# Martinsos/edlib

Measured on AMD Instinct MI355X. Metric: GCUPS (cell updates/s), 1M x 150bp HW reads vs 5Mb target, higher is better.
Workload: dtype u32

## Files before the change

edlib_amd/csrc/engine.hpp:

```cpp
#pragma once
#include "../../include/edlib_amd.h"
#include "common.hpp"
#include "pair_kernels.hpp"
#include "lanepair.hpp"
#include "reads_kernels.hpp"
#include "cross_kernels.hpp"
#include "window_kernels.hpp"
#include "strands.hpp"
#include "flat_pairs_prepare.hpp"
#include "pairs_gather.hpp"

#include <chrono>
#include <deque>
#include <functional>
#include <memory>
#include <vector>

namespace edlib_amd {

struct Tables {
    uint8_t tlut[256];
    uint8_t idToByte[256];
    int sigmaT = 0;
    uint32_t presence[8];
// ... 201 lines not shown
        DevBuf<int> d_best, d_total, d_pos, d_flags;
        DevBuf<uint32_t> d_peq;
        bool zeroCopy = false; PinBuf hostOut;
        std::vector<int> ovfSlots; std::vector<long long> ovfOff; DevBuf<int> d_ovfPool;
        DevBuf<int> d_lvMap, d_lvBest, d_lvCnt, d_lvPos; std::vector<int> lvMap; int lvS = 0, lvCap = 0; bool lvValid = false;
        DevBuf<int> d_list;
        int nreal = -1;
        bool mates = false; DevBuf<int> d_win;
    };
    static constexpr int kLastLevelCap = 16;
    int listOpenSlots(ReadGroup& g, int kDone, std::vector<int>& out);
    DevBuf<uint8_t> d_selTmp_;
    std::vector<std::unique_ptr<ReadGroup>> groups_;
    DevBuf<uint32_t> d_tpk_, d_trows_;
    DevBuf<unsigned long long> d_wordSteps_;
    PinBuf h_wordSteps_; bool wordStepsPending_ = false;
    DevBuf<unsigned long long> d_ringSteps_; PinBuf h_ringSteps_; bool ringStepsUsed_ = false;
    unsigned long long* ringStepsCounter();
    bool banded_ = false;
    int syms_ = 4;
    int packTarget();
    int runReads();
    int makeGroup(const std::vector<int>& units, int words, std::unique_ptr<ReadGroup>& g, long long oneRoundWaves = 0);
    int runGroupScans(ReadGroup& g, bool fullOnly);
    int runGroupExact(ReadGroup& g);
    int collectGroup(ReadGroup& g, std::vector<UnitResult>& res);
    int seedThreshold(const ReadGroup& g, bool fullOnly) const;
    int buildSeedIndex();
    int runSeedPass(ReadGroup& g, int k);
    DevBuf<uint32_t> d_seedCnt_, d_seedOff_, d_seedPos_;
    DevBuf<uint8_t> d_seedTmp_;
    bool hits_ = false, hitsHaveRun_ = false;
    HitListBuffers hitList_;
    HitRows hostHits_;
    DevBuf<int> d_hitSlotUnit_;
    DevBuf<long long> d_hitTotal_;
    int runReadHits();
    int scanGroupHits(ReadGroup& g, int slotBase);
    int hitsScanBanded(ReadGroup& g, int slotBase, const int* d_slotmap, int nlanes, int numSegments, int segLen, int warm);
    struct Piece { long long off; int len; int thr; };
    int scanPieces(const std::vector<Piece>& pieces, bool filter, std::vector<std::pair<int, int>>* cand,
                   std::vector<uint8_t>* overflow, std::vector<int>* best);
    int solveLongReads(std::vector<UnitResult>& res, std::vector<int>& fallback);
    bool filterScan_ = false;
    struct ChainArgs { const uint32_t* in = nullptr; uint32_t* out = nullptr; const int* src = nullptr; int inLanes = 0, blocks = 0; const int* rowBase = nullptr; };
    ChainArgs chain_;
    int solveTallFull(const std::vector<int>& units, std::vector<UnitResult>& res, std::vector<int>& handBack);
    int collectReads(std::vector<UnitResult>& res);
    bool readsCollected_ = true;
    int scanGroup(ReadGroup& g, int mode, const int* d_slotmap, int nlanes, int kcap, const int* d_kinit,
                  int numSegments, int segLen, int warm, int* segBest, int* segCnt, int* segPos, int cap,
                  const long long* posOff, const int* posCap, bool unbanded = false,
                  unsigned long long* wordSteps = nullptr, const uint32_t* peqDense = nullptr,
                  const int* qlenDense = nullptr, int peqBottom = 0, int* liveBest = nullptr);

    DevBuf<PairDesc> d_descs_;
    DevBuf<unsigned long long> d_peq64_;
    DevBuf<StoreEntry> d_store_;
    DevBuf<int> d_aux_, d_out3_, d_outScore_, d_outCount_, d_outLast_, d_posPool_, d_opsLen_, d_alpha_;
    DevBuf<uint8_t> d_ops_;
    DevBuf<long long> d_opsOff_;
    int solve(int mode, bool wantPositions, bool wantPath, const std::vector<UnitSpec>& units, SolveOut& out,
              int ring = 0, int ringH = 1);
    int solveChunk(int mode, bool wantPositions, bool wantPath, const std::vector<UnitSpec>& units,
                   size_t a, size_t b, SolveOut& out, int ring, int ringH);
    static const int kWide = -1;
    static const int kRing32 = -2;
    bool ring32_fits(const std::vector<UnitSpec>& units, size_t a, size_t b, int G) const;
    DevBuf<unsigned long long> d_wide_; DevBuf<unsigned> d_wabort_; PinBuf h_wabort_;
    int wideCap_ = -1;
    struct WidePlan { int slots = 1; size_t perLaunch = 1; };
    int planWide(int mode, PairDesc* descs, size_t n, WidePlan& plan);
    int launchWide(int mode, const PairScanArgs& a, const PairDesc* hostDescs, size_t n, const WidePlan& plan);
    int checkWide();
    bool wideSerial_ = false;
    bool wideGateHeld_ = false;
    void wideGateRelease();
    int solveWideSplit(const std::vector<UnitSpec>& units, std::vector<int>& out, int ring = 0);
    struct KnownSplit { long long qoff; int m; long long toff; int T; int score; int row, left, right; };
    std::vector<KnownSplit> knownSplits_;
    int solveGlobalDistances(const std::vector<UnitSpec>& units, std::vector<int>& score, std::vector<OpsOut>* paths = nullptr);
    int solveSemiGlobal(int mode, bool wantPositions, const std::vector<UnitSpec>& units, SolveOut& out);
    int solveSemiGlobalUnits(int mode, bool wantPositions, const std::vector<UnitSpec>& units, SolveOut& out);
    int solveBanded(const BandLadder& ladder, bool wantPositions, const std::vector<UnitSpec>& units, SolveOut& out);
    int alphabetLengthsBegin(hipEvent_t after = nullptr);
    bool alphaDeferred_ = false;
    int alphabetLengthsEnd(std::vector<UnitResult>& res);
    std::vector<int> alphaUnits_; bool alphaOnHost_ = false, alphaPending_ = false; long long alphaBytes_ = 0;
    hipStream_t side_ = nullptr;
    DevBuf<int> d_alphaIdx_, d_alphaOut_; PinBuf alphaPin_;
    struct PathPiece { long long qoff; int m; long long toff; int T; int score; };
    int hirschbergLevel(const std::vector<PathPiece>& big, std::vector<int>& splitRow,
                        std::vector<int>& leftScore, std::vector<int>& rightScore);
    int solvePaths(const std::vector<PathPiece>& jobs, std::vector<OpsOut>& opsOut, std::vector<int>& status);
    std::vector<std::shared_ptr<PinBuf>> opsKeep_;
    std::deque<std::vector<uint8_t>> opsOwned_;

    int qlen(int u) const { return (int)(qoff_[u + 1] - qoff_[u]); }
    long long tbase(int u) const { return shared_ ? toff_[0] : toff_[u]; }
    int tlen(int u) const { return shared_ ? (int)(toff_[1] - toff_[0]) : (int)(toff_[u + 1] - toff_[u]); }

    void scanTimerStart();
    void scanTimerStop();
    std::vector<std::pair<hipEvent_t, hipEvent_t>> scanEvents_;
    size_t scanEventsUsed_ = 0;

    std::vector<UnitResult> results_, work_;
// ... 151 lines not shown
```

edlib_amd/csrc/engine_reads.hip:

```cpp
#include "engine.hpp"

#include <algorithm>
#include <chrono>
#include <cmath>
#include <condition_variable>
#include <cstring>
#include <mutex>
#include <thread>

namespace edlib_amd {

__global__ void __launch_bounds__(256)
seed_thresholds_kernel(int* __restrict__ kinit, const int* __restrict__ best, const int* __restrict__ cnt, int n)
{
    const int i = blockIdx.x * blockDim.x + threadIdx.x;
    if (i < n && cnt[i] > 0 && best[i] < kinit[i]) kinit[i] = best[i];
}


int Batch::scanGroup(ReadGroup& g, int mode, const int* d_slotmap, int nlanes, int kcap, const int* d_kinit,
                     int numSegments, int segLen, int warm, int* segBest, int* segCnt, int* segPos, int cap,
                     const long long* posOff, const int* posCap, bool unbanded, unsigned long long* wordSteps,
                     const uint32_t* peqDense, const int* qlenDense, int peqBottom, int* liveBest)
{
    ReadScanArgs a{};
    a.peq = peqDense ? peqDense : g.d_peq.p; a.tpk = d_tpk_.p; a.trows = d_trows_.p; a.targetLength = tlen(0);
    if (mode == EDLIB_MODE_SHW) a.targetLength = (int)std::min<long long>(a.targetLength, 64LL * g.nwords + 1);
    a.qlen = qlenDense ? qlenDense : g.d_qlen.p; a.kinit = d_kinit; a.slotmap = d_slotmap; a.nlanes = nlanes;
    a.numSegments = numSegments; a.segLen = segLen; a.warm = warm;
    a.segBest = segBest; a.segCnt = segCnt; a.segPos = segPos; a.cap = cap;
    a.posOff = posOff; a.posCap = posCap;
    a.kcap = kcap; a.wordSteps = wordSteps ? wordSteps : d_wordSteps_.p;
    a.filter = filterScan_ ? 1 : 0;
    a.liveBest = liveBest;
    a.bottomAligned = peqBottom;
    a.chainIn = chain_.in; a.chainOut = chain_.out; a.chainSrc = chain_.src; a.chainInLanes = chain_.inLanes;
    a.chainBlocks = chain_.blocks; a.rowBase = chain_.rowBase;
    const bool chained = chain_.in != nullptr || chain_.out != nullptr;
    static const bool dbg = getenv("EDLIB_AMD_DEBUG") != nullptr;
    if (dbg) {
        EDLIB_AMD_HIP(hipStreamSynchronize(stream_));
        fprintf(stderr, "[edlib_amd] scanGroup nwords=%d mode=%d nlanes=%d S=%d segLen=%d warm=%d cap=%d kcap=%d slotmap=%p posOff=%p rows=%s\n",
                g.nwords, mode, nlanes, numSegments, segLen, warm, cap, kcap, (const void*)d_slotmap, (const void*)posOff,
                peqBottom > 1 ? "delay" : (peqBottom ? "bottom" : "top"));
    }
    scanTimerStart();
    const bool longGroup = g.nwords > kMaxReadWords;
    const long long colsScanned = std::min<long long>(a.targetLength, (long long)numSegments * segLen) + (long long)(numSegments - 1) * warm;
    const bool fullHeight = banded_ && mode == EDLIB_MODE_HW && unbanded && (chained || syms_ > 4 || longGroup);
    const bool bandedKernel = !fullHeight && banded_ && mode == EDLIB_MODE_HW && (!unbanded || syms_ > 4 || longGroup);
    if (peqBottom && (fullHeight || bandedKernel)) EDLIB_AMD_HIP(hipErrorInvalidValue);
    if (fullHeight) {
        EDLIB_AMD_HIP(launch_scan_reads_full(g.nwords, syms_, a, stream_));
        stats.word_steps += (long long)((nlanes + 63) / 64 * 64) * g.nwords * colsScanned;
    } else if (bandedKernel) EDLIB_AMD_HIP(launch_scan_reads_banded(g.nwords, syms_, a, stream_));
    else {
        EDLIB_AMD_HIP(launch_scan_reads(g.nwords, mode, a, stream_));
        stats.word_steps += (long long)((nlanes + 63) / 64 * 64) * g.nwords * colsScanned;
    }
    scanTimerStop();
    if (dbg) {
        EDLIB_AMD_HIP(hipStreamSynchronize(stream_));
        fprintf(stderr, "[edlib_amd] scanGroup done\n");
    }
    return 0;
}

void plan_segments(int nlanes, int T, int mode, int warmFull, long long wantWaves,
                          int& S, int& segLen, int& warm, int minSegCols)
{
    S = 1; segLen = roundup(T, 16); warm = 0;
    if (mode != EDLIB_MODE_HW) return;
    const long long nrblk = ((long long)nlanes + 63) / 64;
    long long want = (wantWaves + nrblk - 1) / nrblk;
    want = std::max(1LL, std::min<long long>(want, std::min(65535, std::max(1, T / minSegCols))));
    if (warmFull > 0) want = std::max(1LL, std::min<long long>(want, std::max<long long>(1, T / (4LL * warmFull))));
    segLen = roundup((int)((T + want - 1) / want), 16);
    S = (T + segLen - 1) / segLen;
    warm = warmFull;
}

int Batch::runReads()
{
    if (groups_.empty()) return 0;
    stats.path |= 1;
    bool seed = false;
    for (auto& gp : groups_) seed = seed || seedThreshold(*gp, false) >= 0;
    if (seed && buildSeedIndex()) return 1;
    for (auto& gp : groups_) if (runGroupScans(*gp, false)) return 1;
    const int mode = (cfg_.mode == EDLIB_MODE_HW || cfg_.mode == EDLIB_MODE_SHW) ? (int)cfg_.mode : (int)EDLIB_MODE_NW;
    for (auto& gp : groups_)
        if (gp->mates) EDLIB_AMD_HIP(launch_resolve_strands(gp->d_perm.p, gp->d_best.p, gp->d_total.p, gp->nslots, mode, cfg_.k,
                                                            gp->d_win.p, stream_));
    for (auto& gp : groups_) if (runGroupExact(*gp)) return 1;
    return 0;
}

int Batch::runGroupScans(ReadGroup& g, bool fullOnly)
{
    const int T = tlen(0);
    const int mode = (cfg_.mode == EDLIB_MODE_HW || cfg_.mode == EDLIB_MODE_SHW) ? (int)cfg_.mode : (int)EDLIB_MODE_NW;
    const bool banded = banded_ && mode == EDLIB_MODE_HW;
    const int kNoCap = 0x3fffffff;
    static const bool dbgLadder = getenv("EDLIB_AMD_DEBUG") != nullptr;
    EDLIB_AMD_HIP(launch_build_peq_reads(g.nwords, syms_, d_qpool_.p, d_qoff_.p, g.d_perm.p, g.nslots,
                                         d_eqtbl_.p, d_presence_.p, cfg_.k, g.d_peq.p, g.d_qlen.p,
                                         g.d_kinit.p, g.d_alphaExtra.p, stream_));
    const int kSeed = seedThreshold(g, fullOnly);
    const int kFirstMax = kSeed >= 0 ? kSeed : std::max(8, g.nwords / 2);
    int kFirst = (kSeed >= 0 && cfg_.k >= 0) ? std::min(kSeed, cfg_.k) : kFirstMax;
    bool twoPass = !fullOnly && banded && (cfg_.k < 0 || cfg_.k > kFirst) && 32 * g.nwords > kFirst;
    std::vector<int> ladder;
    g.lvValid = false;
    auto probe_scan = [&](const std::vector<int>& map, int kc, std::vector<int>& bestOut) -> int {
        const int nm = (int)map.size();
        int S2, segLen2, warm2;
        plan_segments(nm, T, mode, g.warm, 16384, S2, segLen2, warm2);
        const size_t items = (size_t)nm * S2;
        DevBuf<int> d_map, d_sb, d_sc;
        EDLIB_AMD_HIP(d_map.alloc(nm)); EDLIB_AMD_HIP(d_sb.alloc(items)); EDLIB_AMD_HIP(d_sc.alloc(items));
        EDLIB_AMD_HIP(hipMemcpyAsync(d_map.p, map.data(), nm * sizeof(int), hipMemcpyHostToDevice, stream_));
        if (scanGroup(g, mode, d_map.p, nm, kc, g.d_kinit.p, S2, segLen2, warm2,
                      d_sb.p, d_sc.p, d_sb.p , 0, nullptr, nullptr)) return 1;
        std::vector<int> cnts(items), bests(items);
        EDLIB_AMD_HIP(hipMemcpyAsync(cnts.data(), d_sc.p, items * sizeof(int), hipMemcpyDeviceToHost, stream_));
        EDLIB_AMD_HIP(hipMemcpyAsync(bests.data(), d_sb.p, items * sizeof(int), hipMemcpyDeviceToHost, stream_));
        EDLIB_AMD_HIP(hipStreamSynchronize(stream_));
        bestOut.assign(nm, -1);
        for (int i = 0; i < nm; ++i) {
            int b = 0x7fffffff;
            for (int sg = 0; sg < S2; ++sg)
                if (cnts[(size_t)i * S2 + sg] > 0) b = std::min(b, bests[(size_t)i * S2 + sg]);
// ... 41 lines not shown
        if (probe_scan(probe, kFirst, pbest)) return 1;
        int resolved = 0, real = 0;
        std::vector<int> hist(kFirstMax + 1, 0);
        std::vector<int> open;
        for (int i = 0; i < np; ++i) {
            if (g.perm[probe[i]] < 0) continue;
            ++real;
            if (pbest[i] >= 0) { ++resolved; ++hist[pbest[i]]; }
            else if (i == 0 || probe[i] != probe[i - 1]) open.push_back(probe[i]);
        }
        if (resolved > 0) {
            int acc = 0, kq = kFirstMax;
            for (int d = 0; d <= kFirstMax; ++d) { acc += hist[d]; if (acc * 1000LL >= resolved * 995LL) { kq = d; break; } }
            kFirst = std::max(4, std::min(kFirstMax, kq));
        }
        if (real > 0 && resolved * 10 < real * 3) twoPass = false;
        if (twoPass && (int)open.size() * 10 > real && open.size() >= 32 && price_ladder(open, open.size(), real)) return 1;
    }
    std::vector<int> todo;
    bool haveTodo = false;
    if (kSeed >= 0) {
        if (runSeedPass(g, kFirst)) return 1;
        if (twoPass) {
            if (listOpenSlots(g, kFirst, todo)) return 1;
            haveTodo = true;
            if (g.nreal < 0) { g.nreal = 0; for (int u : g.perm) g.nreal += u >= 0; }
            if (g.nslots >= 16384 && todo.size() * 10 > (size_t)g.nreal && todo.size() >= 32) {
                const size_t nsm = std::min<size_t>(2048, todo.size());
                std::vector<int> sample(nsm);
                for (size_t i = 0; i < nsm; ++i) sample[i] = todo[i * todo.size() / nsm];
                if (price_ladder(sample, todo.size(), g.nreal)) return 1;
            }
        }
    } else {
        if (scanGroup(g, mode, nullptr, g.nslots, twoPass ? kFirst : kNoCap, g.d_kinit.p, g.numSegments, g.segLen,
                      g.warm, g.d_segBest.p, g.d_segCnt.p, g.d_segPos.p, 8, nullptr, nullptr, fullOnly)) return 1;
        const bool chained = chain_.in != nullptr || chain_.out != nullptr;
        EDLIB_AMD_HIP(launch_merge_segments(g.d_segBest.p, g.d_segCnt.p, g.d_segPos.p, g.numSegments, 8,
                                            g.nslots, nullptr, 16, g.d_best.p, g.d_total.p, g.d_pos.p,
                                            g.d_flags.p, stream_, chained ? kOvfRescan : kOvfGatherGroup));
    }
    ladder.push_back(kNoCap);
    int kDone = kFirst;
    for (size_t lv = 0; twoPass && lv < ladder.size(); ++lv) {
        const int kcapL = ladder[lv];
        const bool last = kcapL == kNoCap;
        if (!haveTodo && listOpenSlots(g, kDone, todo)) return 1;
        haveTodo = false;
        if (todo.empty()) break;
        {
            const size_t no = todo.size();
            int S2, segLen2, warm2;
            plan_segments((int)no, T, mode, g.warm, 65536, S2, segLen2, warm2);
            const size_t items = no * (size_t)S2;
            const int capL = last ? kLastLevelCap : 8;
            EDLIB_AMD_HIP(g.d_lvMap.ensure(no)); EDLIB_AMD_HIP(g.d_lvBest.ensure(items)); EDLIB_AMD_HIP(g.d_lvCnt.ensure(items));
            EDLIB_AMD_HIP(g.d_lvPos.ensure(items * capL));
            int *d_map = g.d_lvMap.p, *d_sb = g.d_lvBest.p, *d_sc = g.d_lvCnt.p, *d_sp = g.d_lvPos.p;
            EDLIB_AMD_HIP(hipMemcpyAsync(d_map, todo.data(), no * sizeof(int), hipMemcpyHostToDevice, stream_));
            bool plain = false;
            if (last && no >= 4096) {
                const int np2 = 64;
                std::vector<int> sub(np2);
                for (int i = 0; i < np2; ++i) sub[i] = todo[(size_t)((long long)i * no / np2)];
                int S3, segLen3, warm3;
                plan_segments(np2, T, mode, g.warm, 16384, S3, segLen3, warm3);
                const size_t it3 = (size_t)np2 * S3;
                DevBuf<int> d_m3, d_b3, d_c3, d_p3; DevBuf<unsigned long long> d_ws;
                EDLIB_AMD_HIP(d_m3.alloc(np2)); EDLIB_AMD_HIP(d_b3.alloc(it3)); EDLIB_AMD_HIP(d_c3.alloc(it3));
                EDLIB_AMD_HIP(d_p3.alloc(it3 * 8)); EDLIB_AMD_HIP(d_ws.alloc(1));
                EDLIB_AMD_HIP(hipMemcpyAsync(d_m3.p, sub.data(), np2 * sizeof(int), hipMemcpyHostToDevice, stream_));
                EDLIB_AMD_HIP(hipMemsetAsync(d_ws.p, 0, sizeof(unsigned long long), stream_));
                if (scanGroup(g, mode, d_m3.p, np2, kNoCap, g.d_kinit.p, S3, segLen3, warm3,
                              d_b3.p, d_c3.p, d_p3.p, 8, nullptr, nullptr, false, d_ws.p)) return 1;
                unsigned long long ws = 0;
                EDLIB_AMD_HIP(hipMemcpyAsync(&ws, d_ws.p, sizeof ws, hipMemcpyDeviceToHost, stream_));
                EDLIB_AMD_HIP(hipStreamSynchronize(stream_));
                const double cols = (double)np2 * ((double)T + (double)(S3 - 1) * warm3);
                plain = (double)ws >= 0.85 * g.nwords * cols;
                stats.word_steps += (long long)ws;
            }
            const bool bottomOk = plain && mode == EDLIB_MODE_HW && syms_ == 4 && g.nwords <= kMaxReadWords &&
                                  chain_.in == nullptr && chain_.out == nullptr;
            const int bottom = !bottomOk ? 0 : (delay_rows_fit(g.nwords, g.mMax) ? 1 + kDelayRows : 1);
            const size_t no64 = (no + 63) / 64 * 64;
            std::vector<int> perm2(no64, -1);
            for (size_t i = 0; i < no; ++i) perm2[i] = g.perm[todo[i]];
            DevBuf<int> d_perm2, d_qlen2, d_kinit2, d_extra2; DevBuf<uint32_t> d_peq2;
            EDLIB_AMD_HIP(d_perm2.alloc(no64)); EDLIB_AMD_HIP(d_qlen2.alloc(no64)); EDLIB_AMD_HIP(d_kinit2.alloc(no64));
            EDLIB_AMD_HIP(d_extra2.alloc(no64)); EDLIB_AMD_HIP(d_peq2.alloc(no64 * (size_t)syms_ * g.nwords));
            EDLIB_AMD_HIP(hipMemcpyAsync(d_perm2.p, perm2.data(), no64 * sizeof(int), hipMemcpyHostToDevice, stream_));
            EDLIB_AMD_HIP(launch_build_peq_reads(g.nwords, syms_, d_qpool_.p, d_qoff_.p, d_perm2.p, (int)no64,
                                                 d_eqtbl_.p, d_presence_.p, cfg_.k, d_peq2.p, d_qlen2.p,
                                                 d_kinit2.p, d_extra2.p, stream_, bottom));
            const int seedCols = 4096;
            DevBuf<int> d_b0, d_c0, d_p0;
            if (mode == EDLIB_MODE_HW && last && no >= 4096 && S2 > 1 && T >= 16 * seedCols) {
                EDLIB_AMD_HIP(d_b0.alloc(no)); EDLIB_AMD_HIP(d_c0.alloc(no)); EDLIB_AMD_HIP(d_p0.alloc(no * 8));
                if (scanGroup(g, mode, nullptr, (int)no, kcapL, d_kinit2.p, 1, seedCols, 0,
                              d_b0.p, d_c0.p, d_p0.p, 8, nullptr, nullptr, plain, nullptr, d_peq2.p, d_qlen2.p, bottom)) return 1;
                hipLaunchKernelGGL(seed_thresholds_kernel, dim3((unsigned)((no + 255) / 256)), dim3(256), 0, stream_,
                                   d_kinit2.p, d_b0.p, d_c0.p, (int)no);
                EDLIB_AMD_HIP(hipGetLastError());
            }
            DevBuf<int> d_live2;
            if (bottom && S2 > 1) {
                EDLIB_AMD_HIP(d_live2.alloc(no64));
                EDLIB_AMD_HIP(hipMemcpyAsync(d_live2.p, d_kinit2.p, no64 * sizeof(int), hipMemcpyDeviceToDevice, stream_));
            }
            if (scanGroup(g, mode, nullptr, (int)no, kcapL, d_kinit2.p, S2, segLen2, warm2,
                          d_sb, d_sc, d_sp, capL, nullptr, nullptr, plain, nullptr, d_peq2.p, d_qlen2.p, bottom, d_live2.p)) return 1;
            EDLIB_AMD_HIP(launch_merge_segments(d_sb, d_sc, d_sp, S2, capL, (int)no, d_map, 16,
                                                g.d_best.p, g.d_total.p, g.d_pos.p, g.d_flags.p, stream_,
                                                last ? kOvfGatherLevel : kOvfRescan));
            EDLIB_AMD_HIP(hipStreamSynchronize(stream_));
            if (last) { g.lvValid = true; g.lvS = S2; g.lvCap = capL; g.lvMap.swap(todo); }
            if (dbgLadder) fprintf(stderr, "[edlib_amd] level kcap=%d: %zu slots rescanned (plain=%d)\n", kcapL, no, (int)plain);
        }
        kDone = kcapL;
    }
    return 0;
}

int Batch::listOpenSlots(ReadGroup& g, int kDone, std::vector<int>& out)
{
    size_t tmp = 0;
    EDLIB_AMD_HIP(select_slots_scratch_bytes(g.nslots, &tmp));
    EDLIB_AMD_HIP(d_selTmp_.ensure(tmp));
    EDLIB_AMD_HIP(g.d_list.ensure((size_t)g.nslots + 1));
    int* count = g.d_list.p + g.nslots;
    EDLIB_AMD_HIP(launch_select_open_slots(g.d_perm.p, g.d_total.p, g.d_qlen.p, cfg_.k, kDone, g.nslots, g.d_list.p, count,
                                           d_selTmp_.p, d_selTmp_.bytes(), stream_, g.mates));
    int n = 0;
    EDLIB_AMD_HIP(hipMemcpyAsync(&n, count, sizeof(int), hipMemcpyDeviceToHost, stream_));
    EDLIB_AMD_HIP(hipStreamSynchronize(stream_));
    out.resize((size_t)n);
    if (n > 0) {
        EDLIB_AMD_HIP(hipMemcpyAsync(out.data(), g.d_list.p, (size_t)n * sizeof(int), hipMemcpyDeviceToHost, stream_));
        EDLIB_AMD_HIP(hipStreamSynchronize(stream_));
    }
    return 0;
}


int Batch::seedThreshold(const ReadGroup& g, bool fullOnly) const
{
    const long long T = tlen(0);
    if (fullOnly || !banded_ || cfg_.mode != EDLIB_MODE_HW || syms_ != 4 || cfg_.additionalEqualitiesLength > 0 ||
        g.nwords > kMaxReadWords || chain_.in != nullptr || chain_.out != nullptr)
        return -1;
    if (T < 64LL * 32 * g.nwords || g.nslots < 1024 || (long long)g.nslots * T < (1LL << 30)) return -1;
    int kf = -1;
    for (int k = 16; k >= 0 && kf < 0; --k) {
        const int L = g.mMin / (k + 1);
        if (L >= kSeedQ && (double)(k + 1) * (double)T <= std::ldexp(1.0, 2 * L) / 8.0) kf = k;
    }
    return (kf >= 0 && kf >= std::min(8, cfg_.k >= 0 ? cfg_.k : 8)) ? kf : -1;
}

int Batch::buildSeedIndex()
{
    const int T = tlen(0);
    EDLIB_AMD_HIP(d_seedCnt_.ensure((size_t)kSeedBuckets + 1));
    EDLIB_AMD_HIP(d_seedOff_.ensure((size_t)kSeedBuckets + 1));
// ... 350 lines not shown
```

edlib_amd/csrc/reads_kernels.hip:

```cpp
#include "reads_kernels.hpp"
#include "reads_scan.hpp"
#include "reads_column_asm.hpp"

namespace edlib_amd {


__global__ void __launch_bounds__(256)
pack_target_2bit_kernel(const uint8_t* __restrict__ raw, const uint8_t* __restrict__ lut,
                        int T, u32* __restrict__ tpk, int nwords)
{
    __shared__ uint8_t s_lut[256];
    s_lut[threadIdx.x] = lut[threadIdx.x];
    __syncthreads();
    const int w = blockIdx.x * blockDim.x + threadIdx.x;
    if (w >= nwords) return;
    const int base = w * 16;
    u32 out = 0;
    if (base + 16 <= T) {
        const uint4 v = *reinterpret_cast<const uint4*>(raw + base);
        const u32 d[4] = {v.x, v.y, v.z, v.w};
#pragma unroll
        for (int i = 0; i < 16; ++i)
            out |= (u32)(s_lut[(d[i >> 2] >> ((i & 3) * 8)) & 0xFF] & 3) << (2 * i);
    } else {
// ... 133 lines not shown
                                  const u32* tpres, int kcfg, u32* peq, int* qlen, int* kinit,
                                  int* alphaExtra, hipStream_t stream, int bottomAlign)
{
    if (nslots == 0) return hipSuccess;
    if (bottomAlign != 0 && bottomAlign != 1 && bottomAlign != 1 + kDelayRows) return hipErrorInvalidValue;
    if (syms != 4 && syms != 8 && syms != 16) return hipErrorInvalidValue;
    switch (nwords) {
#define CASE(N) case N: return launch_build_peq_t<N>(reads, qoff, perm, nslots, syms, eqtbl, tpres, kcfg, peq, qlen, kinit, alphaExtra, stream, bottomAlign);
        CASE(1) CASE(2) CASE(3) CASE(4) CASE(5) CASE(6) CASE(7) CASE(8) CASE(10) CASE(12) CASE(14) CASE(16) CASE(24) CASE(32)
#undef CASE
    }
    return hipErrorInvalidValue;
}


#define EDLIB_AMD_DISPATCH_COLUMN(sym)                                                     \
    switch (sym) {                                                                         \
        case 0:  column_step<NWD, MODE, BOTTOM>(E0, Pv, Mv, score, sh, zr0, zr1); asm volatile("; sym0"); break; \
        case 1:  column_step<NWD, MODE, BOTTOM>(E1, Pv, Mv, score, sh, zr0, zr1); asm volatile("; sym1"); break; \
        case 2:  column_step<NWD, MODE, BOTTOM>(E2, Pv, Mv, score, sh, zr0, zr1); asm volatile("; sym2"); break; \
        default: column_step<NWD, MODE, BOTTOM>(E3, Pv, Mv, score, sh, zr0, zr1); asm volatile("; sym3"); break; \
    }

#define EDLIB_AMD_DISPATCH_COLUMN_DELAY(FORM, sym)                                         \
    switch (sym) {                                                                         \
        case 0:  column_step_delay<NWD, FORM>(E0, Pv, Mv, score, nph, nmh, zr0, zr1); asm volatile("; sym0"); break; \
        case 1:  column_step_delay<NWD, FORM>(E1, Pv, Mv, score, nph, nmh, zr0, zr1); asm volatile("; sym1"); break; \
        case 2:  column_step_delay<NWD, FORM>(E2, Pv, Mv, score, nph, nmh, zr0, zr1); asm volatile("; sym2"); break; \
        default: column_step_delay<NWD, FORM>(E3, Pv, Mv, score, nph, nmh, zr0, zr1); asm volatile("; sym3"); break; \
    }

#define EDLIB_AMD_TRACK_SCORE(sc, col)                         \
    if ((sc) <= best) {                                        \
        if ((sc) < best) { best = (sc); cnt = 0; }             \
        if (cnt < cap) pos[cnt] = (col);                       \
        ++cnt;                                                 \
    }
#define EDLIB_AMD_TRACK(col) EDLIB_AMD_TRACK_SCORE(score, col)

template <int NWD, int MODE, bool BOTTOM = false, bool DELAY = false>
__global__ void __launch_bounds__(256)
scan_reads_kernel(const ReadScanArgs a)
{
    static_assert(!DELAY || (BOTTOM && MODE == 2), "delay rows: bottom-aligned HW rows");
    constexpr int kHitGroup = 4;
    static_assert(!DELAY || kHitGroup == kDelayRows + 1, "one nibble per group");
    const int lane = threadIdx.x & 63;
    const int rblk = blockIdx.x * 4 + (threadIdx.x >> 6);
    const int seg = blockIdx.y;
    const int idx = rblk * 64 + lane;
    if (rblk * 64 >= a.nlanes) return;
    const bool live = idx < a.nlanes;
    const int slot = live ? (a.slotmap ? a.slotmap[idx] : idx) : 0;

    u32 E0[NWD], E1[NWD], E2[NWD], E3[NWD], Pv[NWD], Mv[NWD];
    {
        const size_t pb = (size_t)(slot >> 6) * 4 * NWD * 64 + (slot & 63);
#pragma unroll
        for (int d = 0; d < NWD; ++d) {
            E0[d] = a.peq[pb + (size_t)(0 * NWD + d) * 64];
            E1[d] = a.peq[pb + (size_t)(1 * NWD + d) * 64];
            E2[d] = a.peq[pb + (size_t)(2 * NWD + d) * 64];
            E3[d] = a.peq[pb + (size_t)(3 * NWD + d) * 64];
            Pv[d] = ~0u;
            Mv[d] = 0u;
        }
    }
    const int m = a.qlen[slot];
    if constexpr (BOTTOM) {
        const int pad = 32 * NWD - (DELAY ? kDelayRows : 0) - m;
#pragma unroll
        for (int d = 0; d < NWD; ++d) {
            const int lo = pad - 32 * d;
            Pv[d] = lo <= 0 ? ~0u : (lo >= 32 ? 0u : ~0u << lo);
        }
    }
    const u32 sh = (u32)(m - 1) & 31u;
    u32 zr0 = 0, zr1 = 0;
    if constexpr (BOTTOM && (NWD == 4 || NWD == 5)) {
        asm volatile("v_mov_b32 %0, 0" : "=v"(zr0));
        asm volatile("v_mov_b32 %0, 0" : "=v"(zr1));
    }
    int score = m;
    int best = a.kinit[slot];
    int cnt = 0;
    const long long item = (long long)idx * a.numSegments + seg;
    const int cap = !live ? 0 : (a.posCap ? a.posCap[item] : a.cap);
    int* pos = a.segPos + (!live ? 0 : (a.posOff ? a.posOff[item] : item * a.cap));
    constexpr int kLiveBlocks = kLivePeriod / 16;
    constexpr int kNoImport = 0x1fffffff;
    int* const livep = BOTTOM ? a.liveBest : nullptr;
    int lidx = idx;
    if constexpr (BOTTOM) asm volatile("" : "+v"(lidx));
#define EDLIB_AMD_LIVE_LOAD() (live ? __hip_atomic_load(livep + lidx, __ATOMIC_RELAXED, __HIP_MEMORY_SCOPE_AGENT) : kNoImport)

    const int T = a.targetLength;
    const int c0 = seg * a.segLen;
    int c1 = c0 + a.segLen; if (c1 > T) c1 = T;
    int cw = c0 - a.warm; if (cw < 0) cw = 0;
    cw &= ~15;

    u32 nph = 0, nmh = 0;
    for (int w = cw >> 4; w < (c0 >> 4); ++w) {
        const u32 tw = a.tpk[w];
#pragma unroll
        for (int j = 0; j < 16; ++j) {
            const u32 sym = (tw >> (2 * j)) & 3u;
            if constexpr (!DELAY) {
                EDLIB_AMD_DISPATCH_COLUMN(sym)
            } else if ((j & (kHitGroup - 1)) != kHitGroup - 1) {
                EDLIB_AMD_DISPATCH_COLUMN_DELAY(0, sym)
            } else {
                EDLIB_AMD_DISPATCH_COLUMN_DELAY(1, sym)
            }
        }
    }
    const int wend = c1 >> 4;
    int lim = best + (kHitGroup - 1);
    if constexpr (DELAY) {
        int lim2 = 2 * best + kHitGroup;
        for (int w0 = c0 >> 4; w0 < wend; w0 += kLiveBlocks) {
        if (livep) {
            const int got = EDLIB_AMD_LIVE_LOAD();
            if (2 * got + kHitGroup < lim2) { lim2 = 2 * got + kHitGroup; cnt = 0; }
        }
        const int w1 = w0 + kLiveBlocks < wend ? w0 + kLiveBlocks : wend;
        for (int w = w0; w < w1; ++w) {
            const u32 tw = a.tpk[w];
#pragma unroll
            for (int j = 0; j < 16; j += kHitGroup) {
#pragma unroll
                for (int q = 0; q < kHitGroup - 1; ++q) {
                    const u32 sym = (tw >> (2 * (j + q))) & 3u;
                    EDLIB_AMD_DISPATCH_COLUMN_DELAY(0, sym)
                }
                const int before = score;
                {
                    const u32 sym = (tw >> (2 * (j + kHitGroup - 1))) & 3u;
                    EDLIB_AMD_DISPATCH_COLUMN_DELAY(1, sym)
                }
                if (__builtin_expect(score + before <= lim2, 0)) {
                    int sc[kHitGroup], acc = before, least = 0x7fffffff;
#pragma unroll
                    for (int q = 0; q < kHitGroup; ++q) {
                        acc += (int)((nph >> (kHitGroup - 1 - q)) & 1u) - (int)((nmh >> (kHitGroup - 1 - q)) & 1u);
                        sc[q] = acc;
                        least = acc < least ? acc : least;
                    }
                    best = (lim2 - kHitGroup) >> 1;
                    if (least <= best) {
#pragma unroll
// ... 3 lines not shown
                    }
                }
            }
        }
        }
        lim = ((lim2 - kHitGroup) >> 1) + (kHitGroup - 1);
    }
    for (int w0 = c0 >> 4; !DELAY && w0 < wend; w0 += kLiveBlocks) {
    if (livep) {
        const int got = EDLIB_AMD_LIVE_LOAD();
        if (got + (kHitGroup - 1) < lim) { lim = got + (kHitGroup - 1); cnt = 0; }
    }
    const int w1 = w0 + kLiveBlocks < wend ? w0 + kLiveBlocks : wend;
    for (int w = w0; w < w1; ++w) {
        const u32 tw = a.tpk[w];
#pragma unroll
        for (int j = 0; j < 16; j += kHitGroup) {
            int sc[kHitGroup];
#pragma unroll
            for (int q = 0; q < kHitGroup; ++q) {
                const u32 sym = (tw >> (2 * (j + q))) & 3u;
                EDLIB_AMD_DISPATCH_COLUMN(sym)
                sc[q] = score;
            }
            if (MODE != 0) {
                if (__builtin_expect(score <= lim, 0)) {
                    best = lim - (kHitGroup - 1);
#pragma unroll
                    for (int q = 0; q < kHitGroup; ++q) { EDLIB_AMD_TRACK_SCORE(sc[q], w * 16 + j + q) }
                    if (livep && live && best + (kHitGroup - 1) < lim) atomicMin(livep + lidx, best);
                    lim = best + (kHitGroup - 1);
                }
            }
        }
    }
    }
#undef EDLIB_AMD_LIVE_LOAD
    best = lim - (kHitGroup - 1);
    const int rem = c1 - (wend << 4);
    if (rem > 0) {
        u32 tw = a.tpk[wend];
        for (int j = 0; j < rem; ++j) {
            const u32 sym = tw & 3u;
            tw >>= 2;
            if constexpr (DELAY) { EDLIB_AMD_DISPATCH_COLUMN_DELAY(2, sym) } else { EDLIB_AMD_DISPATCH_COLUMN(sym) }
            if (MODE != 0) { EDLIB_AMD_TRACK(wend * 16 + j) }
        }
    }
    if (live) {
        const size_t o = (size_t)lidx * a.numSegments + seg;
        a.segBest[o] = (MODE == 0) ? score : best;
        a.segCnt[o] = (MODE == 0) ? 1 : cnt;
    }
}

template <int NWD>
static hipError_t launch_scan_mode(int mode, const ReadScanArgs& a, hipStream_t stream)
{
    const int nrblk = (a.nlanes + 63) / 64;
    dim3 grid((nrblk + 3) / 4, a.numSegments), block(256);
    switch (mode) {
        case 0: hipLaunchKernelGGL((scan_reads_kernel<NWD, 0>), grid, block, 0, stream, a); break;
        case 1: hipLaunchKernelGGL((scan_reads_kernel<NWD, 1>), grid, block, 0, stream, a); break;
        case 2: if (a.bottomAligned == 1 + kDelayRows) hipLaunchKernelGGL((scan_reads_kernel<NWD, 2, true, true>), grid, block, 0, stream, a);
                else if (a.bottomAligned) hipLaunchKernelGGL((scan_reads_kernel<NWD, 2, true>), grid, block, 0, stream, a);
                else hipLaunchKernelGGL((scan_reads_kernel<NWD, 2>), grid, block, 0, stream, a);
                break;
        default: return hipErrorInvalidValue;
    }
    return hipGetLastError();
}

hipError_t launch_scan_reads(int nwords, int mode, const ReadScanArgs& a, hipStream_t stream)
{
    if (a.nlanes == 0) return hipSuccess;
    if (a.bottomAligned && mode != 2) return hipErrorInvalidValue;
    if (a.bottomAligned != 0 && a.bottomAligned != 1 && a.bottomAligned != 1 + kDelayRows) return hipErrorInvalidValue;
    switch (nwords) {
#define CASE(N) case N: return launch_scan_mode<N>(mode, a, stream);
        CASE(1) CASE(2) CASE(3) CASE(4) CASE(5) CASE(6) CASE(7) CASE(8)
#undef CASE
    }
    return hipErrorInvalidValue;
}


hipError_t launch_scan_reads_full_long(int nwords, int syms, const ReadScanArgs& a, hipStream_t stream);
hipError_t launch_scan_reads_banded_long(int nwords, int syms, const ReadScanArgs& a, hipStream_t stream);

template <int S, bool CHAIN>
static hipError_t launch_scan_reads_full_s(int nwords, const ReadScanArgs& a, hipStream_t stream)
{
    dim3 grid((a.nlanes + 63) / 64, a.numSegments), block(64);
    switch (nwords) {
#define CASE(N) case N: EDLIB_AMD_CHECK_STATIC_LDS((scan_reads_full_kernel<N, S, CHAIN>), N * S * 256); \
                        hipLaunchKernelGGL((scan_reads_full_kernel<N, S, CHAIN>), grid, block, 0, stream, a); break;
        CASE(1) CASE(2) CASE(3) CASE(4) CASE(5) CASE(6) CASE(7) CASE(8)
#undef CASE
        default: return hipErrorInvalidValue;
    }
    return hipGetLastError();
}

hipError_t launch_scan_reads_full(int nwords, int syms, const ReadScanArgs& a, hipStream_t stream)
{
    if (a.nlanes == 0) return hipSuccess;
    if (nwords > kMaxReadWords) return launch_scan_reads_full_long(nwords, syms, a, stream);
    const bool chain = a.chainIn != nullptr || a.chainOut != nullptr;
    switch (syms) {
        case 4: return chain ? launch_scan_reads_full_s<4, true>(nwords, a, stream) : launch_scan_reads_full_s<4, false>(nwords, a, stream);
        case 8: return chain ? launch_scan_reads_full_s<8, true>(nwords, a, stream) : launch_scan_reads_full_s<8, false>(nwords, a, stream);
        case 16: return chain ? launch_scan_reads_full_s<16, true>(nwords, a, stream) : launch_scan_reads_full_s<16, false>(nwords, a, stream);
    }
    return hipErrorInvalidValue;
}

template <int S>
static hipError_t launch_scan_reads_banded_s(int nwords, const ReadScanArgs& a, hipStream_t stream)
{
    const int nrblk = (a.nlanes + 63) / 64;
    dim3 grid(nrblk, a.numSegments), block(64);
    switch (nwords) {
#define CASE(N) case N: if (a.filter) { EDLIB_AMD_CHECK_STATIC_LDS((scan_reads_banded_kernel<N, S, true>), N * S * 256); \
                                            hipLaunchKernelGGL((scan_reads_banded_kernel<N, S, true>), grid, block, 0, stream, a); } \
                        else { EDLIB_AMD_CHECK_STATIC_LDS((scan_reads_banded_kernel<N, S, false>), N * S * 256); \
                               hipLaunchKernelGGL((scan_reads_banded_kernel<N, S, false>), grid, block, 0, stream, a); } break;
        CASE(1) CASE(2) CASE(3) CASE(4) CASE(5) CASE(6) CASE(7) CASE(8)
#undef CASE
        default: return hipErrorInvalidValue;
    }
    return hipGetLastError();
}

hipError_t launch_scan_reads_banded(int nwords, int syms, const ReadScanArgs& a, hipStream_t stream)
{
    if (a.nlanes == 0) return hipSuccess;
    if (nwords > kMaxReadWords) return a.filter ? hipErrorInvalidValue : launch_scan_reads_banded_long(nwords, syms, a, stream);
    switch (syms) {
        case 4: return launch_scan_reads_banded_s<4>(nwords, a, stream);
        case 8: return launch_scan_reads_banded_s<8>(nwords, a, stream);
        case 16: return launch_scan_reads_banded_s<16>(nwords, a, stream);
    }
    return hipErrorInvalidValue;
}


__global__ void __launch_bounds__(256)
collect_candidates_kernel(const int* __restrict__ segCnt, const int* __restrict__ segPos, int S, int cap, int nlanes,
                          int* __restrict__ out, int maxOut, int* __restrict__ counter, int* __restrict__ overflow)
{
    const long long item = (long long)blockIdx.x * blockDim.x + threadIdx.x;
    if (item >= (long long)nlanes * S) return;
    const int c = segCnt[item];
    if (c <= 0) return;
    const int lane = (int)(item / S);
    if (c > cap) overflow[lane] = 1;
    const int take = c < cap ? c : cap;
    const int at = atomicAdd(counter, take);
    for (int i = 0; i < take; ++i)
        if (at + i < maxOut) { out[2 * (at + i)] = lane; out[2 * (at + i) + 1] = segPos[item * cap + i]; }
}

hipError_t launch_collect_candidates(const int* segCnt, const int* segPos, int numSegments, int cap, int nlanes,
                                     int* out, int maxOut, int* counter, int* overflow, hipStream_t stream)
{
    const long long items = (long long)nlanes * numSegments;
    if (items == 0) return hipSuccess;
    hipLaunchKernelGGL(collect_candidates_kernel, dim3((unsigned)((items + 255) / 256)), dim3(256), 0, stream,
                       segCnt, segPos, numSegments, cap, nlanes, out, maxOut, counter, overflow);
    return hipGetLastError();
}


__global__ void __launch_bounds__(256)
merge_segments_kernel(const int* __restrict__ segBest, const int* __restrict__ segCnt,
                      const int* __restrict__ segPos, int S, int cap, int nlanes,
                      const int* __restrict__ slotmap, int capFinal,
                      int* __restrict__ best, int* __restrict__ total, int* __restrict__ pos,
                      int* __restrict__ flags, int gatherFlag)
{
    const int idx = blockIdx.x * blockDim.x + threadIdx.x;
    if (idx >= nlanes) return;
    const int slot = slotmap ? slotmap[idx] : idx;
    const size_t base = (size_t)idx * S;
    int b = 0x7fffffff;
    for (int s = 0; s < S; ++s)
        if (segCnt[base + s] > 0 && segBest[base + s] < b) b = segBest[base + s];
    int n = 0, ovf = 0;
    if (b != 0x7fffffff) {
// ... 107 lines not shown
```

edlib_amd/csrc/reads_kernels.hpp:

```cpp
#pragma once
#include <hip/hip_runtime.h>
#include <stdint.h>

#include "hit_list.hpp"

namespace edlib_amd {

constexpr int kMaxReadWords = 8;
constexpr int kMaxLongReadWords = 16;
constexpr int kMaxLongReadWords4 = 32;
constexpr int kFilterFromWords = 13;
inline int read_group_words(int m) { const int w = (m + 31) / 32; return w <= kMaxReadWords ? w : (w <= 10 ? 10 : (w <= 12 ? 12 : (w <= 14 ? 14 : (w <= 16 ? 16 : (w <= 24 ? 24 : 32))))); }
constexpr int kDelayRows = 3;
constexpr bool delay_rows_fit(int nwords, int longest) { return nwords <= kMaxReadWords && longest >= 1 && longest + kDelayRows <= 32 * nwords; }
constexpr int kLanes = 64;


struct ReadScanArgs {
    const uint32_t* peq;
    const uint32_t* tpk;
    const uint32_t* trows;
    int targetLength;
    const int* qlen;
    const int* kinit;
    const int* slotmap;
    int nlanes;
    int numSegments;
    int segLen;
    int warm;
    int* segBest;
    int* segCnt;
    int* segPos;
    int cap;
    const long long* posOff;
    const int* posCap;
    int kcap;
    unsigned long long* wordSteps;
    const uint32_t* chainIn; uint32_t* chainOut;
    const int* chainSrc;
    int chainInLanes;
    int chainBlocks;
    const int* rowBase;
    int filter;
    HitList hits;
    int slotBase;
    int bottomAligned;
    int* liveBest;
};
constexpr int kLivePeriod = 1024;

hipError_t launch_scan_reads(int nwords, int mode, const ReadScanArgs& a, hipStream_t stream);

hipError_t launch_scan_reads_banded(int nwords, int syms, const ReadScanArgs& a, hipStream_t stream);

hipError_t launch_scan_reads_full(int nwords, int syms, const ReadScanArgs& a, hipStream_t stream);

hipError_t launch_pack_target_2bit(const uint8_t* raw, const uint8_t* lut, int targetLength,
                                   uint32_t* tpk, hipStream_t stream);
hipError_t launch_pack_target_rows(const uint8_t* raw, const uint8_t* lut, int targetLength,
                                   uint32_t* trows, int ndwords, hipStream_t stream);

hipError_t launch_build_peq_reads(int nwords, int syms, const uint8_t* reads, const long long* qoff,
                                  const int* perm, int nslots, const uint16_t* eqtbl,
                                  const uint32_t* targetPresence , int kcfg,
                                  uint32_t* peq, int* qlen, int* kinit, int* alphaExtra,
                                  hipStream_t stream, int bottomAlign = 0);

hipError_t launch_collect_candidates(const int* segCnt, const int* segPos, int numSegments, int cap, int nlanes,
                                     int* out, int maxOut, int* counter, int* overflow, hipStream_t stream);

constexpr int kSeedQ = 12;
constexpr int kSeedBuckets = 1 << (2 * kSeedQ);
constexpr int kSeedBucketCap = 64;
constexpr int kSeedMaxDiag = 32;
constexpr int kSeedMaxWindow = 1024;

struct SeedArgs {
    const uint32_t* peq;
    const int* qlen;
    const int* perm;
    const uint32_t* tpk;
    int targetLength;
    const uint32_t* seedOff;
    const uint32_t* seedPos;
    int nslots;
    int k;
    int* best; int* total; int* pos; int* flags;
    int* backSlots; int* backCount;
    unsigned long long* wordSteps;
    HitList hits;
    int slotBase;
};

hipError_t seed_index_scratch_bytes(size_t* bytes);
hipError_t launch_build_seed_index(const uint32_t* tpk, int targetLength, uint32_t* cnt, uint32_t* off, uint32_t* pos,
                                   void* tmp, size_t tmpBytes, hipStream_t stream);
hipError_t launch_seed_verify(int nwords, const SeedArgs& a, hipStream_t stream);

hipError_t launch_merge_segments(const int* segBest, const int* segCnt, const int* segPos,
                                 int numSegments, int cap, int nlanes, const int* slotmap, int capFinal,
                                 int* best, int* total, int* pos, int* flags, hipStream_t stream, int gatherFlag = 1);
constexpr int kOvfRescan = 1, kOvfGatherLevel = 2, kOvfGatherGroup = 4;
hipError_t launch_gather_segments(const int* segBest, const int* segCnt, const int* segPos, int numSegments, int cap, int n,
                                  const int* idx, const long long* off, const int* lim, int* out, hipStream_t stream);
// ... 15 lines not shown
```

Before: 3.312 million.

## Taper segment lengths in bottom-aligned read scan to shrink tail drain

Adds a per-segment table so the last-level bottom-aligned read scan can use variable segment lengths. Segments shrink as the remaining target columns fall, sized from the GPU's resident workgroup count, so the final waves of the grid finish closer together. The aim is to cut idle time at the end of the kernel, at the cost of more segments and therefore more warm-up overlap and merge work. It also adds optional wave-clock diagnostics that are compiled out by default.

```diff
diff --git a/edlib_amd/csrc/engine.hpp b/edlib_amd/csrc/engine.hpp
--- a/edlib_amd/csrc/engine.hpp
+++ b/edlib_amd/csrc/engine.hpp
@@ -277,7 +277,8 @@
                   int numSegments, int segLen, int warm, int* segBest, int* segCnt, int* segPos, int cap,
                   const long long* posOff, const int* posCap, bool unbanded = false,
                   unsigned long long* wordSteps = nullptr, const uint32_t* peqDense = nullptr,
-                  const int* qlenDense = nullptr, int peqBottom = 0, int* liveBest = nullptr);
+                  const int* qlenDense = nullptr, int peqBottom = 0, int* liveBest = nullptr,
+                  const Segment* segTable = nullptr, long long tableCols = 0);
 
     DevBuf<PairDesc> d_descs_;
     DevBuf<unsigned long long> d_peq64_;
diff --git a/edlib_amd/csrc/engine_reads.hip b/edlib_amd/csrc/engine_reads.hip
--- a/edlib_amd/csrc/engine_reads.hip
+++ b/edlib_amd/csrc/engine_reads.hip
@@ -21,7 +21,8 @@
 int Batch::scanGroup(ReadGroup& g, int mode, const int* d_slotmap, int nlanes, int kcap, const int* d_kinit,
                      int numSegments, int segLen, int warm, int* segBest, int* segCnt, int* segPos, int cap,
                      const long long* posOff, const int* posCap, bool unbanded, unsigned long long* wordSteps,
-                     const uint32_t* peqDense, const int* qlenDense, int peqBottom, int* liveBest)
+                     const uint32_t* peqDense, const int* qlenDense, int peqBottom, int* liveBest,
+                     const Segment* segTable, long long tableCols)
 {
     ReadScanArgs a{};
     a.peq = peqDense ? peqDense : g.d_peq.p; a.tpk = d_tpk_.p; a.trows = d_trows_.p; a.targetLength = tlen(0);
@@ -33,6 +34,7 @@
     a.kcap = kcap; a.wordSteps = wordSteps ? wordSteps : d_wordSteps_.p;
     a.filter = filterScan_ ? 1 : 0;
     a.liveBest = liveBest;
+    a.segTable = segTable;
     a.bottomAligned = peqBottom;
     a.chainIn = chain_.in; a.chainOut = chain_.out; a.chainSrc = chain_.src; a.chainInLanes = chain_.inLanes;
     a.chainBlocks = chain_.blocks; a.rowBase = chain_.rowBase;
@@ -46,7 +48,18 @@
     }
     scanTimerStart();
     const bool longGroup = g.nwords > kMaxReadWords;
-    const long long colsScanned = std::min<long long>(a.targetLength, (long long)numSegments * segLen) + (long long)(numSegments - 1) * warm;
+    const long long colsScanned = segTable ? tableCols
+        : std::min<long long>(a.targetLength, (long long)numSegments * segLen) + (long long)(numSegments - 1) * warm;
+#ifdef EDLIB_AMD_DRAIN_DIAG
+    const char* drainOut = (peqBottom && liveBest) ? "edlib_amd_drain.bin" : nullptr;
+    DevBuf<unsigned long long> d_clk;
+    const size_t drainGX = ((size_t)(nlanes + 63) / 64 + 3) / 4, drainWaves = drainGX * numSegments * 4;
+    if (drainOut) {
+        EDLIB_AMD_HIP(d_clk.alloc(2 * drainWaves));
+        EDLIB_AMD_HIP(hipMemsetAsync(d_clk.p, 0, 2 * drainWaves * sizeof(unsigned long long), stream_));
+        a.waveClock = d_clk.p;
+    }
+#endif
     const bool fullHeight = banded_ && mode == EDLIB_MODE_HW && unbanded && (chained || syms_ > 4 || longGroup);
     const bool bandedKernel = !fullHeight && banded_ && mode == EDLIB_MODE_HW && (!unbanded || syms_ > 4 || longGroup);
     if (peqBottom && (fullHeight || bandedKernel)) EDLIB_AMD_HIP(hipErrorInvalidValue);
@@ -59,6 +72,17 @@
         stats.word_steps += (long long)((nlanes + 63) / 64 * 64) * g.nwords * colsScanned;
     }
     scanTimerStop();
+#ifdef EDLIB_AMD_DRAIN_DIAG
+    if (drainOut) {
+        std::vector<unsigned long long> clk(2 * drainWaves);
+        EDLIB_AMD_HIP(hipMemcpyAsync(clk.data(), d_clk.p, clk.size() * sizeof(unsigned long long), hipMemcpyDeviceToHost, stream_));
+        EDLIB_AMD_HIP(hipStreamSynchronize(stream_));
+        if (FILE* f = fopen(drainOut, "wb")) {
+            const unsigned long long head[2] = {drainGX, (unsigned long long)numSegments};
+            fwrite(head, sizeof head, 1, f); fwrite(clk.data(), sizeof(unsigned long long), clk.size(), f); fclose(f);
+        }
+    }
+#endif
     if (dbg) {
         EDLIB_AMD_HIP(hipStreamSynchronize(stream_));
         fprintf(stderr, "[edlib_amd] scanGroup done\n");
@@ -69,15 +93,7 @@
 void plan_segments(int nlanes, int T, int mode, int warmFull, long long wantWaves,
                           int& S, int& segLen, int& warm, int minSegCols)
 {
-    S = 1; segLen = roundup(T, 16); warm = 0;
-    if (mode != EDLIB_MODE_HW) return;
-    const long long nrblk = ((long long)nlanes + 63) / 64;
-    long long want = (wantWaves + nrblk - 1) / nrblk;
-    want = std::max(1LL, std::min<long long>(want, std::min(65535, std::max(1, T / minSegCols))));
-    if (warmFull > 0) want = std::max(1LL, std::min<long long>(want, std::max<long long>(1, T / (4LL * warmFull))));
-    segLen = roundup((int)((T + want - 1) / want), 16);
-    S = (T + segLen - 1) / segLen;
-    warm = warmFull;
+    plan_segments_uniform(nlanes, T, mode == EDLIB_MODE_HW, warmFull, wantWaves, minSegCols, S, segLen, warm);
 }
 
 int Batch::runReads()
@@ -225,11 +241,9 @@
             const size_t no = todo.size();
             int S2, segLen2, warm2;
             plan_segments((int)no, T, mode, g.warm, 65536, S2, segLen2, warm2);
-            const size_t items = no * (size_t)S2;
             const int capL = last ? kLastLevelCap : 8;
-            EDLIB_AMD_HIP(g.d_lvMap.ensure(no)); EDLIB_AMD_HIP(g.d_lvBest.ensure(items)); EDLIB_AMD_HIP(g.d_lvCnt.ensure(items));
-            EDLIB_AMD_HIP(g.d_lvPos.ensure(items * capL));
-            int *d_map = g.d_lvMap.p, *d_sb = g.d_lvBest.p, *d_sc = g.d_lvCnt.p, *d_sp = g.d_lvPos.p;
+            EDLIB_AMD_HIP(g.d_lvMap.ensure(no));
+            int* d_map = g.d_lvMap.p;
             EDLIB_AMD_HIP(hipMemcpyAsync(d_map, todo.data(), no * sizeof(int), hipMemcpyHostToDevice, stream_));
             bool plain = false;
             if (last && no >= 4096) {
@@ -256,6 +270,24 @@
             const bool bottomOk = plain && mode == EDLIB_MODE_HW && syms_ == 4 && g.nwords <= kMaxReadWords &&
                                   chain_.in == nullptr && chain_.out == nullptr;
             const int bottom = !bottomOk ? 0 : (delay_rows_fit(g.nwords, g.mMax) ? 1 + kDelayRows : 1);
+            std::vector<Segment> table;
+            DevBuf<Segment> d_segTable; long long tableCols = 0;
+            if (bottom && S2 > 1 && no >= 4096) {
+                int resident = 0;
+                EDLIB_AMD_HIP(scan_reads_resident_workgroups(g.nwords, bottom, &resident));
+#ifdef EDLIB_AMD_DRAIN_UNIFORM
+                resident = 0;
+#endif
+                table = plan_segments_tapered(T, (int)(((no + 63) / 64 + 3) / 4), resident, warm2, segLen2);
+                S2 = (int)table.size();
+                for (const Segment& sg : table) tableCols += sg.cols + std::min(warm2, sg.start);
+                EDLIB_AMD_HIP(d_segTable.alloc(table.size()));
+                EDLIB_AMD_HIP(hipMemcpyAsync(d_segTable.p, table.data(), table.size() * sizeof(Segment), hipMemcpyHostToDevice, stream_));
+            }
+            const size_t items = no * (size_t)S2;
+            EDLIB_AMD_HIP(g.d_lvBest.ensure(items)); EDLIB_AMD_HIP(g.d_lvCnt.ensure(items));
+            EDLIB_AMD_HIP(g.d_lvPos.ensure(items * capL));
+            int *d_sb = g.d_lvBest.p, *d_sc = g.d_lvCnt.p, *d_sp = g.d_lvPos.p;
             const size_t no64 = (no + 63) / 64 * 64;
             std::vector<int> perm2(no64, -1);
             for (size_t i = 0; i < no; ++i) perm2[i] = g.perm[todo[i]];
@@ -282,7 +314,8 @@
                 EDLIB_AMD_HIP(hipMemcpyAsync(d_live2.p, d_kinit2.p, no64 * sizeof(int), hipMemcpyDeviceToDevice, stream_));
             }
             if (scanGroup(g, mode, nullptr, (int)no, kcapL, d_kinit2.p, S2, segLen2, warm2,
-                          d_sb, d_sc, d_sp, capL, nullptr, nullptr, plain, nullptr, d_peq2.p, d_qlen2.p, bottom, d_live2.p)) return 1;
+                          d_sb, d_sc, d_sp, capL, nullptr, nullptr, plain, nullptr, d_peq2.p, d_qlen2.p, bottom, d_live2.p,
+                          d_segTable.p, tableCols)) return 1;
             EDLIB_AMD_HIP(launch_merge_segments(d_sb, d_sc, d_sp, S2, capL, (int)no, d_map, 16,
                                                 g.d_best.p, g.d_total.p, g.d_pos.p, g.d_flags.p, stream_,
                                                 last ? kOvfGatherLevel : kOvfRescan));
diff --git a/edlib_amd/csrc/reads_kernels.hip b/edlib_amd/csrc/reads_kernels.hip
--- a/edlib_amd/csrc/reads_kernels.hip
+++ b/edlib_amd/csrc/reads_kernels.hip
@@ -209,6 +209,10 @@
     if (rblk * 64 >= a.nlanes) return;
     const bool live = idx < a.nlanes;
     const int slot = live ? (a.slotmap ? a.slotmap[idx] : idx) : 0;
+#ifdef EDLIB_AMD_DRAIN_DIAG
+    if (BOTTOM && a.waveClock && lane == 0)
+        a.waveClock[((size_t)blockIdx.y * gridDim.x + blockIdx.x) * 4 + (threadIdx.x >> 6)] = wall_clock64();
+#endif
 
     u32 E0[NWD], E1[NWD], E2[NWD], E3[NWD], Pv[NWD], Mv[NWD];
     {
@@ -252,8 +256,9 @@
 #define EDLIB_AMD_LIVE_LOAD() (live ? __hip_atomic_load(livep + lidx, __ATOMIC_RELAXED, __HIP_MEMORY_SCOPE_AGENT) : kNoImport)
 
     const int T = a.targetLength;
-    const int c0 = seg * a.segLen;
-    int c1 = c0 + a.segLen; if (c1 > T) c1 = T;
+    int c0 = seg * a.segLen, c1 = c0 + a.segLen;
+    if (a.segTable) { const Segment sg = a.segTable[seg]; c0 = sg.start; c1 = c0 + sg.cols; }
+    if (c1 > T) c1 = T;
     int cw = c0 - a.warm; if (cw < 0) cw = 0;
     cw &= ~15;
 
@@ -363,6 +368,12 @@
         a.segBest[o] = (MODE == 0) ? score : best;
         a.segCnt[o] = (MODE == 0) ? 1 : cnt;
     }
+#ifdef EDLIB_AMD_DRAIN_DIAG
+    if (BOTTOM && a.waveClock && __builtin_amdgcn_mbcnt_hi(~0u, __builtin_amdgcn_mbcnt_lo(~0u, 0u)) == 0) {
+        const int rb = lidx >> 6;
+        a.waveClock[((size_t)gridDim.y + blockIdx.y) * gridDim.x * 4 + rb] = wall_clock64();
+    }
+#endif
 }
 
 template <int NWD>
@@ -395,6 +406,29 @@
     return hipErrorInvalidValue;
 }
 
+template <int NWD>
+static hipError_t resident_bottom(int bottomAligned, int* perCU)
+{
+    if (bottomAligned == 1 + kDelayRows) return hipOccupancyMaxActiveBlocksPerMultiprocessor(perCU, scan_reads_kernel<NWD, 2, true, true>, 256, 0);
+    return hipOccupancyMaxActiveBlocksPerMultiprocessor(perCU, scan_reads_kernel<NWD, 2, true>, 256, 0);
+}
+
+hipError_t scan_reads_resident_workgroups(int nwords, int bottomAligned, int* resident)
+{
+    int dev = 0, cus = 0, perCU = 0;
+    hipError_t e = hipGetDevice(&dev);
+    if (e == hipSuccess) e = hipDeviceGetAttribute(&cus, hipDeviceAttributeMultiprocessorCount, dev);
+    if (e != hipSuccess) return e;
+    switch (nwords) {
+#define CASE(N) case N: e = resident_bottom<N>(bottomAligned, &perCU); break;
+        CASE(1) CASE(2) CASE(3) CASE(4) CASE(5) CASE(6) CASE(7) CASE(8)
+#undef CASE
+        default: return hipErrorInvalidValue;
+    }
+    *resident = perCU * cus;
+    return e;
+}
+
 
 hipError_t launch_scan_reads_full_long(int nwords, int syms, const ReadScanArgs& a, hipStream_t stream);
 hipError_t launch_scan_reads_banded_long(int nwords, int syms, const ReadScanArgs& a, hipStream_t stream);
@@ -416,6 +450,7 @@
 hipError_t launch_scan_reads_full(int nwords, int syms, const ReadScanArgs& a, hipStream_t stream)
 {
     if (a.nlanes == 0) return hipSuccess;
+    if (a.segTable) return hipErrorInvalidValue;
     if (nwords > kMaxReadWords) return launch_scan_reads_full_long(nwords, syms, a, stream);
     const bool chain = a.chainIn != nullptr || a.chainOut != nullptr;
     switch (syms) {
@@ -446,6 +481,7 @@
 hipError_t launch_scan_reads_banded(int nwords, int syms, const ReadScanArgs& a, hipStream_t stream)
 {
     if (a.nlanes == 0) return hipSuccess;
+    if (a.segTable) return hipErrorInvalidValue;
     if (nwords > kMaxReadWords) return a.filter ? hipErrorInvalidValue : launch_scan_reads_banded_long(nwords, syms, a, stream);
     switch (syms) {
         case 4: return launch_scan_reads_banded_s<4>(nwords, a, stream);
diff --git a/edlib_amd/csrc/reads_kernels.hpp b/edlib_amd/csrc/reads_kernels.hpp
--- a/edlib_amd/csrc/reads_kernels.hpp
+++ b/edlib_amd/csrc/reads_kernels.hpp
@@ -3,6 +3,7 @@
 #include <stdint.h>
 
 #include "hit_list.hpp"
+#include "segment_plan.hpp"
 
 namespace edlib_amd {
 
@@ -46,10 +47,15 @@
     int slotBase;
     int bottomAligned;
     int* liveBest;
+    const Segment* segTable;
+#ifdef EDLIB_AMD_DRAIN_DIAG
+    unsigned long long* waveClock;
+#endif
 };
 constexpr int kLivePeriod = 1024;
 
 hipError_t launch_scan_reads(int nwords, int mode, const ReadScanArgs& a, hipStream_t stream);
+hipError_t scan_reads_resident_workgroups(int nwords, int bottomAligned, int* resident);
 
 hipError_t launch_scan_reads_banded(int nwords, int syms, const ReadScanArgs& a, hipStream_t stream);
 
diff --git a/edlib_amd/csrc/segment_plan.hpp b/edlib_amd/csrc/segment_plan.hpp
--- /dev/null
+++ b/edlib_amd/csrc/segment_plan.hpp
@@ -0,0 +1,55 @@
+#pragma once
+#include <algorithm>
+#include <vector>
+
+namespace edlib_amd {
+
+struct Segment { int start, cols; };
+
+constexpr int kMaxSegments = 65535;
+
+inline int seg_roundup16(long long x) { return (int)((x + 15) / 16 * 16); }
+
+inline void plan_segments_uniform(int nlanes, int T, bool hw, int warmFull, long long wantWaves, int minSegCols,
+                                  int& S, int& segLen, int& warm)
+{
+    S = 1; segLen = seg_roundup16(T); warm = 0;
+    if (!hw) return;
+    const long long nrblk = ((long long)nlanes + 63) / 64;
+    long long want = (wantWaves + nrblk - 1) / nrblk;
+    want = std::max(1LL, std::min<long long>(want, std::min(kMaxSegments, std::max(1, T / minSegCols))));
+    if (warmFull > 0) want = std::max(1LL, std::min<long long>(want, std::max<long long>(1, T / (4LL * warmFull))));
+    segLen = seg_roundup16((T + want - 1) / want);
+    S = (T + segLen - 1) / segLen;
+    warm = warmFull;
+}
+
+inline std::vector<Segment> uniform_segment_table(int T, int Lmax)
+{
+    std::vector<Segment> t;
+    for (long long c = 0; c < T; c += Lmax) t.push_back({(int)c, (int)std::min<long long>(Lmax, T - c)});
+    return t;
+}
+
+inline std::vector<Segment> plan_segments_tapered(int T, int gridX, int resident, int warm, int Lmax)
+{
+    Lmax = std::max(16, Lmax / 16 * 16);
+    int minCols = std::max(16, seg_roundup16(4LL * warm));
+    minCols = std::max(minCols, seg_roundup16(((long long)T + kMaxSegments - 2) / (kMaxSegments - 1)));
+    const long long uniformS = ((long long)T + Lmax - 1) / Lmax;
+    if (T <= 0 || gridX <= 0 || resident <= 0 || Lmax <= minCols || uniformS * gridX < 2LL * resident)
+        return uniform_segment_table(T, Lmax);
+    std::vector<Segment> t;
+    long long c = 0;
+    while (c < T) {
+        const long long rem = T - c;
+        long long len = rem * gridX / (2LL * resident) / 16 * 16;
+        len = std::max<long long>(minCols, std::min<long long>(Lmax, len));
+        if (len > rem) len = rem;
+        t.push_back({(int)c, (int)len});
+        c += len;
+    }
+    return t;
+}
+
+}
```

After: 3.382 million (median of 6 runs). +2.1%, better.
